# yukara-ikemiya/friendly-stable-audio-tools

Measured on AMD Instinct MI355X. Metric: audio-seconds/sec @44.1kHz stereo, 100-step DPM++, SA-Open-1.0 shape, higher is better.
Workload: dtype fp16; 1 GPU; Stable-Audio-Open-1.0 DiT shape (24 layers, D=1536, S=1025, CFG 7 -> 2 sequences/prompt) + Oobleck decode, 1 prompt(s)/GPU x 47.55 s, 100 DPM-Solver++(3M) SDE steps; prompts_per_gpu=1, codec_dtype=fp16, sampler_steps=100, layernorm=fused, cross_attention=fused, sample_size=2097152, parallelism=dp1 (rank-strided prompts, one all-gather)

## Files before the change

friendly-stable-audio-tools_amd/csrc/gemm_ph8.hip:

```cpp
#include <algorithm>
#include <type_traits>

#include "sat_common.h"

namespace {

typedef __attribute__((address_space(3))) void* lds_void_p;
typedef float f32x4_t __attribute__((ext_vector_type(4)));

template <int N>
__device__ __forceinline__ void wait_lgkmcnt() {
    asm volatile("s_waitcnt lgkmcnt(%0)" ::"n"(N) : "memory");
}

__device__ __forceinline__ float silu_fast(float x) { return x * __builtin_amdgcn_rcpf(1.0f + __expf(-x)); }

__device__ __forceinline__ unsigned lds_addr(const void* p) {
    return (unsigned)(size_t)(__attribute__((address_space(3))) const char*)(const char*)p;
}
__device__ __forceinline__ float lds_ld32(const void* p) {
    float v;
    asm volatile("ds_read_b32 %0, %1" : "=v"(v) : "v"(lds_addr(p)) : "memory");
    return v;
}
// ... 4 lines not shown
}
__device__ __forceinline__ f32x4_t lds_ld128(const void* p) {
    f32x4_t v;
    asm volatile("ds_read_b128 %0, %1" : "=v"(v) : "v"(lds_addr(p)) : "memory");
    return v;
}
__device__ __forceinline__ void lds_st64(void* p, float2 v) { asm volatile("ds_write_b64 %0, %1" ::"v"(lds_addr(p)), "v"(v) : "memory"); }
__device__ __forceinline__ void lds_st128(void* p, f32x4_t v) { asm volatile("ds_write_b128 %0, %1" ::"v"(lds_addr(p)), "v"(v) : "memory"); }
__device__ __forceinline__ void lds_tie() {}
template <typename T, typename... Ts>
__device__ __forceinline__ void lds_tie(T& v, Ts&... vs) {
    asm volatile("" : "+v"(v));
    lds_tie(vs...);
}
template <typename... Ts>
__device__ __forceinline__ void lds_wait(Ts&... vs) {
    asm volatile("s_waitcnt lgkmcnt(0)" ::: "memory");
    lds_tie(vs...);
}

template <int PERM>
__device__ __forceinline__ int chan_of(int ni, int nf, int i) {
    const int q = i >> 2, r = i & 3;
    if constexpr (PERM == 0) return ni * 32 + nf * 16 + i;
    else if constexpr (PERM == 1) return ni * 32 + q * 8 + nf * 4 + r;
    else return ni == 0 ? nf * 16 + i : 32 + q * 8 + nf * 4 + r;
}

struct Seg {
    int m0, n0;
    int kt0, nk;
    bool whole;
    bool tr;
};

struct Ph8F32Epi {
    __amdgpu_buffer_rsrc_t rsC, rsXb, rsPart;
    int ldc, N;
    bool accumulate, prod;
    const float* gate;
    int gate_rows, gate_ld, M;
};
__device__ __forceinline__ Ph8F32Epi ph8_f32_epi(const GemmArgs& g) {
    Ph8F32Epi e;
    e.rsC = __builtin_amdgcn_make_buffer_rsrc((void*)g.C, 0, (int)((unsigned)g.M * (unsigned)g.ldc * 4u), 0x00020000);
    e.rsXb = __builtin_amdgcn_make_buffer_rsrc((void*)g.xb, 0, g.xb ? (int)((unsigned)g.M * (unsigned)g.N * 2u) : 0, 0x00020000);
    e.rsPart = __builtin_amdgcn_make_buffer_rsrc((void*)g.ln_part_out, 0, g.ln_part_out ? (int)((unsigned)g.M * (unsigned)(g.N >> 6) * 8u) : 0, 0x00020000);
    e.ldc = g.ldc; e.N = g.N; e.accumulate = g.accumulate != 0; e.prod = g.xb != nullptr;
    e.gate = g.gate; e.gate_rows = g.gate_rows; e.gate_ld = g.gate_ld; e.M = g.M;
    return e;
}
typedef unsigned int ph8_u32x4 __attribute__((ext_vector_type(4)));
typedef unsigned int ph8_u32x2 __attribute__((ext_vector_type(2)));
__device__ __forceinline__ void ph8_load_resid(const Ph8F32Epi& e, f32x4_t (&old)[4], int m, int ncol0, int q4) {
    const int off = (m * e.ldc + ncol0 + 4 * q4) * 4;
#pragma unroll
    for (int nb = 0; nb < 4; ++nb)
        old[nb] = __builtin_bit_cast(f32x4_t, __builtin_amdgcn_raw_buffer_load_b128(e.rsC, off + nb * 64, 0, 0));
}
template <bool RT, bool PROD_C>
__device__ __forceinline__ void ph8_epi_f32_row(const Ph8F32Epi& e, f32x4_t (&v)[4], const f32x4_t (&old)[4], int m, int ncol0, int q4) {
    const int off = (m * e.ldc + ncol0 + 4 * q4) * 4;
    [[maybe_unused]] const float* grow = nullptr;
    bool prod = PROD_C;
    if constexpr (RT) {
        prod = e.prod;
// ... 6 lines not shown
#pragma unroll
    for (int nb = 0; nb < 4; ++nb) {
        f32x4_t x = v[nb];
        if constexpr (RT) {
            if (grow) x *= *reinterpret_cast<const f32x4_t*>(grow + nb * 16);
        }
        const f32x4_t o = old[nb];
        x += e.accumulate ? o : f32x4_t{0.f, 0.f, 0.f, 0.f};
        __builtin_amdgcn_raw_buffer_store_b128(__builtin_bit_cast(ph8_u32x4, x), e.rsC, off + nb * 64, 0, 0);
        if (prod) {
            opx4 xr;
#pragma unroll
            for (int k = 0; k < 4; ++k) {
                xr[k] = f32_to_op(x[k]);
                const float f = op_to_f32(xr[k]);
                sum += f;
                sq += f * f;
            }
            __builtin_amdgcn_raw_buffer_store_b64(__builtin_bit_cast(ph8_u32x2, xr), e.rsXb, (m * e.N + ncol0 + 4 * q4 + nb * 16) * 2, 0, 0);
        }
    }
    if (prod) {
        sum += __int_as_float(__builtin_amdgcn_ds_swizzle(__float_as_int(sum), 0x401F));
        sq += __int_as_float(__builtin_amdgcn_ds_swizzle(__float_as_int(sq), 0x401F));
        u32x2 a = __builtin_amdgcn_permlane32_swap(__float_as_uint(sum), __float_as_uint(sum), false, false);
        u32x2 b = __builtin_amdgcn_permlane32_swap(__float_as_uint(sq), __float_as_uint(sq), false, false);
        sum = __uint_as_float(a[0]) + __uint_as_float(a[1]);
        sq = __uint_as_float(b[0]) + __uint_as_float(b[1]);
        const int poff = q4 == 0 ? (m * (e.N >> 6) + (ncol0 >> 6)) * 8 : 0x7ffffff0;
        __builtin_amdgcn_raw_buffer_store_b64(ph8_u32x2{__float_as_uint(sum), __float_as_uint(sq)}, e.rsPart, poff, 0, 0);
    }
}

template <int EPI, int DBG = 0, int FP8 = 0, bool GATED = false>
__global__ __launch_bounds__(512) void gemm_ph8_kernel(GemmArgs g, Ph8Sched sc, unsigned long long* ts = nullptr) {
    sat_f16_saturate();
    constexpr int WN = 4, MFQ = 4;
    constexpr int NW = 2 * WN, NT = NW * 64;
    constexpr int QR = MFQ * 16;
    constexpr int WR = 2 * QR;
    constexpr int BM = 2 * WR, BN = WN * 64;
    constexpr int MB = 2 * MFQ;
    constexpr int AH = (BM / 2) * 128, WH = (BN / 2) * 128;
    static_assert(NT / 2 == BM, "two threads per row in the LayerNorm prologue");
    [[maybe_unused]] int ts_n = 0;
    constexpr int BUF_BYTES = 2 * (AH + WH), RING_BYTES = 2 * BUF_BYTES;
    auto koff = [](int kind) { return kind == 0 ? 0 : kind == 1 ? WH : kind == 2 ? WH + AH : 2 * WH + AH; };
    extern __shared__ __attribute__((aligned(16))) char smem[];

    const int tid_ = threadIdx.x;
    const int lane = tid_ & 63;
    const int wave = __builtin_amdgcn_readfirstlane(tid_ >> 6);
    const int wr = wave / WN, wc = wave % WN;
    const int l15_ = lane & 15, q4_ = lane >> 4;
    const int M = g.M, N = g.N, K = g.K;
    const int wgi = xcd_remap(blockIdx.x, sc.G);

    auto tile_of = [&](int id, int& tm, int& tn) { ph8_tile_of(sc, id, tm, tn); };
    int dp_s = 0;
    int sk_b = 0, sk_e = 0;
    if (sc.sk_tiles) ph8_wg_units(sc, wgi, sk_b, sk_e);
    int sk_u = sk_b;
    auto next_seg = [&](Seg& s) -> bool {
        int tm, tn;
        if (dp_s < sc.dp_rounds) {
            tile_of(dp_s * sc.G + wgi, tm, tn);
            ++dp_s;
            s.kt0 = 0; s.nk = 2 * sc.nkp; s.whole = true;
        } else {
            if (sk_u >= sk_e) return false;
            const int j = sk_u / sc.nkp;
            const int ub = sk_u - j * sc.nkp;
            const int ue = min(sc.nkp, ub + (sk_e - sk_u));
            tile_of(sc.rem0 + j, tm, tn);
            s.kt0 = 2 * ub; s.nk = 2 * (ue - ub); s.whole = (ub == 0 && ue == sc.nkp);
            sk_u += ue - ub;
        }
        s.m0 = tm * BM; s.n0 = tn * BN;
        s.tr = true;
        if constexpr (EPI == EPI_HEADS) s.tr = !(g.heads.kind[s.n0 / (g.heads.heads * 64)] & 1);
        return true;
    };

    const __amdgpu_buffer_rsrc_t rsA = __builtin_amdgcn_make_buffer_rsrc((void*)g.A, 0, (int)((unsigned)M * (unsigned)K * 2u), 0x00020000);
    __amdgpu_buffer_rsrc_t rsW = rsA;
    int voffA[2], voffW[2][2];
    auto setup_dma = [&](const Seg& s) {
        int lane_l = lane;
        asm volatile("" : "+v"(lane_l));
        rsW = __builtin_amdgcn_make_buffer_rsrc((void*)(g.W + (size_t)s.n0 * K), 0, BN * K * 2, 0x00020000);
        const int sub = lane_l >> 3, pos = lane_l & 7;
#pragma unroll
        for (int i = 0; i < 2; ++i) {
            const int r = i * (NW * 8) + wave * 8 + sub;
            const int c = pos ^ ((r >> 1) & 7);
            voffA[i] = (s.m0 + (r / QR) * WR + (r % QR)) * (K * 2) + c * 16;
            const int wcol = r >> 5, nf = (r >> 4) & 1, fi = r & 15;
#pragma unroll
            for (int ni = 0; ni < 2; ++ni) {
                int ch;
                if constexpr (EPI == EPI_F32) ch = chan_of<0>(ni, nf, fi);
                else if constexpr (EPI == EPI_SWIGLU) ch = chan_of<1>(ni, nf, fi);
                else ch = s.tr ? chan_of<2>(ni, nf, fi) : chan_of<0>(ni, nf, fi);
                voffW[ni][i] = (wcol * 64 + ch) * (K * 2) + c * 16;
            }
        }
    };
    const int hiA = QR * K * 2;
    auto issue = [&](int kind, int buf, int kt) {
        char* dst = smem + buf * BUF_BYTES + koff(kind) + wave * 1024;
        const int soff = __builtin_amdgcn_readfirstlane(kt * 128);
#pragma unroll
        for (int i = 0; i < 2; ++i) {
            if (kind & 1)
                __builtin_amdgcn_raw_ptr_buffer_load_lds(rsA, (lds_void_p)(dst + i * (NW * 1024)), 16, voffA[i] + (kind == 3 ? hiA : 0), soff, 0, 0);
            else
                __builtin_amdgcn_raw_ptr_buffer_load_lds(rsW, (lds_void_p)(dst + i * (NW * 1024)), 16, voffW[kind >> 1][i], soff, 0, 0);
        }
    };

    const int swz = l15_ >> 1;
    [[maybe_unused]] const int swz_ = swz;
    int offA[2], offW[2];
#pragma unroll
    for (int ks = 0; ks < 2; ++ks) {
        const int ch = ((ks * 4 + q4_) ^ swz) << 4;
        offA[ks] = (wr * QR + l15_) * 128 + ch;
        offW[ks] = (wc * 32 + l15_) * 128 + ch;
    }

    f32x4_t acc[MB][4];
    opx8 fa[MFQ][2], fwl[2][2], fwh[2][2];
    typedef int i32x8_t __attribute__((ext_vector_type(8)));
    [[maybe_unused]] i32x8_t fa8[MFQ], fw8l[2], fw8h[2];
    [[maybe_unused]] const int off8[2] = {(((2 * q4_) ^ swz_) << 4), (((2 * q4_ + 1) ^ swz_) << 4)};
    auto read8 = [&](const char* rowbase) -> i32x8_t {
        const u32x4 lo = *reinterpret_cast<const u32x4*>(rowbase + off8[0]);
        const u32x4 hi = *reinterpret_cast<const u32x4*>(rowbase + off8[1]);
        return i32x8_t{(int)lo[0], (int)lo[1], (int)lo[2], (int)lo[3], (int)hi[0], (int)hi[1], (int)hi[2], (int)hi[3]};
    };
    [[maybe_unused]] auto read_a8 = [&](int buf, int hi) {
        const char* base = smem + buf * BUF_BYTES + koff(hi ? 3 : 1) + (wr * QR + l15_) * 128;
#pragma unroll
        for (int f = 0; f < MFQ; ++f) fa8[f] = read8(base + f * 2048);
    };
    [[maybe_unused]] auto read_w8 = [&](int buf, int hi, i32x8_t (&fw)[2]) {
        const char* base = smem + buf * BUF_BYTES + koff(hi ? 2 : 0) + (wc * 32 + l15_) * 128;
#pragma unroll
        for (int f = 0; f < 2; ++f) fw[f] = read8(base + f * 2048);
    };
    auto read_a = [&](int buf, int hi) {
        const char* base = smem + buf * BUF_BYTES + koff(hi ? 3 : 1);
#pragma unroll
        for (int f = 0; f < MFQ; ++f)
#pragma unroll
            for (int ks = 0; ks < 2; ++ks) fa[f][ks] = *reinterpret_cast<const opx8*>(base + offA[ks] + f * 2048);
    };
    auto read_w = [&](int buf, int hi, opx8 (&fw)[2][2]) {
        const char* base = smem + buf * BUF_BYTES + koff(hi ? 2 : 0);
#pragma unroll
        for (int f = 0; f < 2; ++f)
#pragma unroll
            for (int ks = 0; ks < 2; ++ks) fw[f][ks] = *reinterpret_cast<const opx8*>(base + offW[ks] + f * 2048);
    };

    auto main_loop = [&](auto swap_c, const int kt0, const int nk, const bool q_valid0, const bool q_valid1) {
        constexpr bool SWAP = decltype(swap_c)::value;
        auto mfma_half = [&](int mi, int ni_first) {
            if (!(mi ? q_valid1 : q_valid0)) return;
            __builtin_amdgcn_s_setprio(1);
            if constexpr (FP8 != 0) {
#pragma unroll
                for (int h = 0; h < 2; ++h) {
                    const int ni = ni_first ^ h;
                    i32x8_t (&fw)[2] = ni ? fw8h : fw8l;
#pragma unroll
                    for (int f = 0; f < MFQ; ++f)
#pragma unroll
                        for (int n = 0; n < 2; ++n)
                            acc[mi * MFQ + f][ni * 2 + n] =
                                SWAP ? __builtin_amdgcn_mfma_scale_f32_16x16x128_f8f6f4(fw[n], fa8[f], acc[mi * MFQ + f][ni * 2 + n], 0, 0, 0, 0x7F7F7F7F, 0, 0x7F7F7F7F)
                                     : __builtin_amdgcn_mfma_scale_f32_16x16x128_f8f6f4(fa8[f], fw[n], acc[mi * MFQ + f][ni * 2 + n], 0, 0, 0, 0x7F7F7F7F, 0, 0x7F7F7F7F);
                }
                __builtin_amdgcn_s_setprio(0);
                return;
            }
#pragma unroll
            for (int h = 0; h < 2; ++h) {
                const int ni = ni_first ^ h;
                opx8 (&fw)[2][2] = ni ? fwh : fwl;
#pragma unroll
                for (int ks = 0; ks < 2; ++ks)
#pragma unroll
                    for (int f = 0; f < MFQ; ++f)
#pragma unroll
                        for (int n = 0; n < 2; ++n)
                            acc[mi * MFQ + f][ni * 2 + n] = SWAP ? mfma_16x16x32(fw[n][ks], fa[f][ks], acc[mi * MFQ + f][ni * 2 + n])
                                                                 : mfma_16x16x32(fa[f][ks], fw[n][ks], acc[mi * MFQ + f][ni * 2 + n]);
            }
            __builtin_amdgcn_s_setprio(0);
        };
        auto k_tile = [&](auto buf_c, auto mode_c, int t) {
            constexpr int BUF = decltype(buf_c)::value;
            constexpr int MODE = decltype(mode_c)::value;
            if constexpr (FP8 != 0) {
                read_w8(BUF, 0, fw8l);
                read_w8(BUF, 1, fw8h);
                read_a8(BUF, 0);
            } else {
                read_w(BUF, 0, fwl);
                read_w(BUF, 1, fwh);
                read_a(BUF, 0);
            }
            if constexpr (MODE <= 1) {
                issue(2, BUF ^ 1, t + 1);
                issue(3, BUF ^ 1, t + 1);
                wait_vmcnt<8>();
            } else {
                wait_vmcnt<0>();
            }
            __builtin_amdgcn_sched_barrier(0);
            wait_lgkmcnt<0>();
            __builtin_amdgcn_s_barrier();
            __builtin_amdgcn_sched_barrier(0);
            mfma_half(0, 0);
            __builtin_amdgcn_sched_barrier(0);
            __builtin_amdgcn_s_barrier();
            if constexpr (FP8 != 0) read_a8(BUF, 1);
            else read_a(BUF, 1);
            if constexpr (MODE == 0) {
                issue(0, BUF, t + 2);
                issue(1, BUF, t + 2);
                wait_vmcnt<6>();
// ... 113 lines not shown

    struct RopePre {
        f32x4_t cs, sn;
    };
    constexpr int ROPE16_OFF = RING_BYTES + 2 * LN_BYTES;
    if constexpr (EPI == EPI_HEADS) {
        if (tid_ < 32 && g.heads.rope_cos) {
            const int r16 = g.heads.S > 16 ? 16 : g.heads.S - 1;
            reinterpret_cast<float*>(smem + ROPE16_OFF)[tid_] = (tid_ < 16 ? g.heads.rope_cos : g.heads.rope_sin)[r16 * 16 + (tid_ & 15)];
        }
    }
    constexpr int PRO_DMA = 2 * (4 + PRO_T1);
    static_assert(PRO_DMA == 12, "prologue = 6 half-tiles");
    [[maybe_unused]] auto rope_load = [&](f32x4_t& cs, f32x4_t& sn, int row, int q4) {
        const unsigned voff = (unsigned)(row * 16 + 4 * q4) * 4u;
        asm volatile("global_load_dwordx4 %0, %1, %2" : "=v"(cs) : "v"(voff), "s"(g.heads.rope_cos) : "memory");
        asm volatile("global_load_dwordx4 %0, %1, %2" : "=v"(sn) : "v"(voff), "s"(g.heads.rope_sin) : "memory");
    };
    [[maybe_unused]] auto rope_prefetch = [&](const Seg& s, RopePre& rp) {
        int l15 = l15_, q4 = q4_;
        asm volatile("" : "+v"(l15), "+v"(q4));
        const int S = g.heads.S;
        const int m = s.m0 + wr * WR + l15;
        rope_load(rp.cs, rp.sn, (m < M ? m : M - 1) % S, q4);
    };
    [[maybe_unused]] auto rope_wait = [](auto n_c, RopePre& rp) {
        wait_vmcnt<decltype(n_c)::value>();
        asm volatile("" : "+v"(rp.cs), "+v"(rp.sn));
    };

    auto epilogue = [&](const Seg& s, int lb, [[maybe_unused]] RopePre& rp, [[maybe_unused]] const bool dma_behind) {
        int l15 = l15_, q4 = q4_;
        asm volatile("" : "+v"(l15), "+v"(q4));
        const int mrow0 = s.m0 + wr * WR + l15;
        const int ncol0 = s.n0 + wc * 64;
        [[maybe_unused]] const float2* ln = reinterpret_cast<const float2*>(smem + RING_BYTES + lb * LN_BYTES) + wr * WR;
        [[maybe_unused]] const float* lc1 = reinterpret_cast<const float*>(smem + RING_BYTES + lb * LN_BYTES + BM * 8) + wc * 64;
        [[maybe_unused]] const float* lc2 = lc1 + BN;
        if constexpr (EPI == EPI_F32) {
            const Ph8F32Epi fe = ph8_f32_epi(g);
            auto run = [&](auto rt_c, auto prod_c) {
                constexpr bool RT = decltype(rt_c)::value, PROD = decltype(prod_c)::value;
                f32x4_t old[2][2][4];
#pragma unroll
                for (int i = 0; i < 2; ++i) ph8_load_resid(fe, old[0][i], mrow0 + i * 16, ncol0, q4);
#pragma unroll
                for (int h = 0; h < MB / 2; ++h) {
                    if (h + 1 < MB / 2) {
#pragma unroll
                        for (int i = 0; i < 2; ++i) ph8_load_resid(fe, old[(h + 1) & 1][i], mrow0 + ((h + 1) * 2 + i) * 16, ncol0, q4);
                    }
                    __builtin_amdgcn_sched_barrier(0);
#pragma unroll
                    for (int i = 0; i < 2; ++i) ph8_epi_f32_row<RT, PROD>(fe, acc[h * 2 + i], old[h & 1][i], mrow0 + (h * 2 + i) * 16, ncol0, q4);
                    __builtin_amdgcn_sched_barrier(0);
                }
            };
            if constexpr (GATED) run(std::true_type{}, std::false_type{});
            else run(std::false_type{}, std::true_type{});
        } else if constexpr (EPI == EPI_SWIGLU) {
            const int ldh = N >> 1;
            f32x4_t c1v[2], c1g[2], c2v[2], c2g[2];
#pragma unroll
            for (int nf = 0; nf < 2; ++nf) {
                c1v[nf] = lds_ld128(lc1 + q4 * 8 + nf * 4);
                c1g[nf] = lds_ld128(lc1 + 32 + q4 * 8 + nf * 4);
                c2v[nf] = lds_ld128(lc2 + q4 * 8 + nf * 4);
                c2g[nf] = lds_ld128(lc2 + 32 + q4 * 8 + nf * 4);
            }
            float2 stv[MB];
#pragma unroll
            for (int mb = 0; mb < MB; ++mb) stv[mb] = lds_ld64(ln + mb * 16 + l15);
            lds_wait(c1v[0], c1v[1], c1g[0], c1g[1], c2v[0], c2v[1], c2g[0], c2g[1]);
#pragma unroll
            for (int mb = 0; mb < MB; ++mb) lds_tie(stv[mb]);
            const __amdgpu_buffer_rsrc_t rsH = __builtin_amdgcn_make_buffer_rsrc((void*)g.H, 0, (int)((unsigned)M * (unsigned)ldh * 2u), 0x00020000);
            const int hcol = (ncol0 >> 1) + q4 * 8;
#pragma unroll
            for (int mb = 0; mb < MB; ++mb) {
                const int m = mrow0 + mb * 16;
                const float2 st = stv[mb];
                unsigned pk[4];
                [[maybe_unused]] float hv8[8];
#pragma unroll
                for (int nf = 0; nf < 2; ++nf) {
                    float hv[4];
#pragma unroll
                    for (int e = 0; e < 4; ++e) {
                        const float v = fold(acc[mb][nf][e], st.x, st.y, c1v[nf][e], c2v[nf][e]);
                        const float gt = fold(acc[mb][2 + nf][e], st.x, st.y, c1g[nf][e], c2g[nf][e]);
                        hv[e] = v * silu_fast(gt);
                        if constexpr (FP8 != 0) hv8[4 * nf + e] = hv[e];
                    }
                    pk[2 * nf] = pack_op2(hv[0], hv[1]);
                    pk[2 * nf + 1] = pack_op2(hv[2], hv[3]);
                }
                if constexpr (FP8 != 0) {
                    if (g.H8) {
                        float am = 0.f;
#pragma unroll
                        for (int i = 0; i < 8; ++i) am = fmaxf(am, fabsf(hv8[i]));
                        am = m < M ? am : 0.f;
                        am = fmaxf(am, __int_as_float(__builtin_amdgcn_ds_swizzle(__float_as_int(am), 0x401F)));
                        am = fmaxf(am, __int_as_float(__builtin_amdgcn_ds_bpermute((lane ^ 32) << 2, __float_as_int(am))));
                        const float t = am * (1.0f / 448.0f);
                        const unsigned tb = __float_as_uint(t);
                        int e = (int)((tb >> 23) & 0xff) - 127 + ((tb & 0x7fffff) ? 1 : 0);
                        e = am > 0.f ? (e < -127 ? -127 : (e > 127 ? 127 : e)) : -127;
                        const float inv = __uint_as_float((unsigned)(127 - e) << 23);
                        unsigned q0 = __builtin_amdgcn_cvt_pk_fp8_f32(hv8[0] * inv, hv8[1] * inv, 0u, false);
                        q0 = __builtin_amdgcn_cvt_pk_fp8_f32(hv8[2] * inv, hv8[3] * inv, q0, true);
                        unsigned q1 = __builtin_amdgcn_cvt_pk_fp8_f32(hv8[4] * inv, hv8[5] * inv, 0u, false);
                        q1 = __builtin_amdgcn_cvt_pk_fp8_f32(hv8[6] * inv, hv8[7] * inv, q1, true);
                        if (m < M) {
                            *reinterpret_cast<u32x2*>(g.H8 + (size_t)m * ldh + (ncol0 >> 1) + q4 * 8) = u32x2{q0, q1};
                            if (q4 == 0) g.Hs[(size_t)m * (ldh >> 5) + (ncol0 >> 6)] = (unsigned char)(e + 127);
                        }
                        continue;
                    }
                }
                __builtin_amdgcn_raw_buffer_store_b128(ph8_u32x4{pk[0], pk[1], pk[2], pk[3]}, rsH, (m * ldh + hcol) * 2, 0, 0);
            }
        } else {
            const HeadsEpi& he = g.heads;
            const int hp = he.heads * 64;
            const int part = ncol0 / hp;
            const int head = (ncol0 - part * hp) >> 6;
            const int kind = he.kind[part];
            op_t* __restrict__ dst = he.out[part];
            const int S = he.S, Spad = he.Spad;
            if (s.tr) {
                f32x4_t c1[4], c2[4];
#pragma unroll
                for (int nf = 0; nf < 2; ++nf) {
                    c1[nf] = lds_ld128(lc1 + nf * 16 + 4 * q4);
                    c2[nf] = lds_ld128(lc2 + nf * 16 + 4 * q4);
                    c1[2 + nf] = lds_ld128(lc1 + 32 + q4 * 8 + nf * 4);
                    c2[2 + nf] = lds_ld128(lc2 + 32 + q4 * 8 + nf * 4);
                }
                float2 stv[2];
                stv[0] = lds_ld64(ln + l15);
                [[maybe_unused]] f32x4_t c16 = lds_ld128(smem + ROPE16_OFF + 16 * q4), s16 = lds_ld128(smem + ROPE16_OFF + 64 + 16 * q4);
                lds_wait(c1[0], c1[1], c1[2], c1[3], c2[0], c2[1], c2[2], c2[3], c16, s16, stv[0]);
                int b = 0, sq_ = 0;
                {
                    const int mc = mrow0 < M ? mrow0 : M - 1;
                    b = mc / S;
                    sq_ = mc - b * S;
                }
                if (kind & 2) {
                    if (dma_behind) rope_wait(std::integral_constant<int, PRO_DMA>{}, rp);
                    else rope_wait(std::integral_constant<int, 0>{}, rp);
                }
#pragma unroll
// ... 113 lines not shown
    prepare_finish(cur, lb, lnpre);
    while (true) {
        {
            f32x4_t b0[4] = {{0.f, 0.f, 0.f, 0.f}, {0.f, 0.f, 0.f, 0.f}, {0.f, 0.f, 0.f, 0.f}, {0.f, 0.f, 0.f, 0.f}};
            if constexpr (EPI == EPI_F32) {
                if (g.bias && cur.whole) {
                    int q4 = q4_;
                    asm volatile("" : "+v"(q4));
#pragma unroll
                    for (int j = 0; j < 4; ++j) b0[j] = *reinterpret_cast<const f32x4_t*>(g.bias + cur.n0 + wc * 64 + 4 * q4 + j * 16);
                }
            }
#pragma unroll
            for (int i = 0; i < MB; ++i)
#pragma unroll
                for (int j = 0; j < 4; ++j) acc[i][j] = b0[j];
        }
        if constexpr (EPI != EPI_HEADS) {
#pragma unroll
            for (int i = 0; i < MB; ++i)
#pragma unroll
                for (int j = 0; j < 4; ++j) asm volatile("" : "+v"(acc[i][j]));
        }
        if constexpr (EPI_STORES >= 0) {
            if (stores_behind) wait_vmcnt<6 + (EPI_STORES >= 0 ? EPI_STORES : 0)>();
            else wait_vmcnt<6>();
        } else {
            wait_vmcnt<0>();
        }
        wait_lgkmcnt<0>();
        __builtin_amdgcn_s_barrier();
        [[maybe_unused]] unsigned long long t0 = 0, t1 = 0, t2 = 0;
        if constexpr (DBG == 9) t0 = __builtin_amdgcn_s_memrealtime();
        const int mq = cur.m0 + wr * WR;
        const bool rows_valid = mq < M;
        if (cur.tr) main_loop(std::true_type{}, cur.kt0, cur.nk, rows_valid, mq + QR < M);
        else main_loop(std::false_type{}, cur.kt0, cur.nk, rows_valid, mq + QR < M);
        if constexpr (DBG == 9) t1 = __builtin_amdgcn_s_memrealtime();
        const bool more = next_seg(nxt);
        [[maybe_unused]] RopePre rp;
        if constexpr (EPI == EPI_HEADS) {
            if (rows_valid && cur.tr && (g.heads.kind[cur.n0 / (g.heads.heads * 64)] & 2)) rope_prefetch(cur, rp);
        }
        if (more) {
            prepare_issue(nxt, lnpre);
            if constexpr (!LN_DEFER) prepare_finish(nxt, lb ^ 1, lnpre);
        }
        bool fin = true;
        if (EPI == EPI_F32 && !cur.whole) {
            int lane_l = lane;
            asm volatile("" : "+v"(lane_l));
            float* mine = sc.sk_slab + (size_t)wgi * (BM * BN) + (size_t)(wave * MB * 4) * 256 + lane_l * 4;
#pragma unroll
            for (int mb = 0; mb < MB; ++mb)
#pragma unroll
                for (int nb = 0; nb < 4; ++nb) *reinterpret_cast<f32x4_t*>(mine + (mb * 4 + nb) * 256) = acc[mb][nb];
            fin = false;
        }
        if constexpr (DBG == 9) t2 = __builtin_amdgcn_s_memrealtime();
        if (fin && rows_valid) epilogue(cur, lb, rp, more);
        stores_behind = fin && rows_valid;
        if constexpr (DBG == 9) {
            if (tid_ == 0 && ts_n < 4) {
                unsigned long long* o = ts + ((size_t)blockIdx.x * 4 + ts_n) * 8;
                o[0] = t0; o[1] = t1; o[2] = t2; o[3] = __builtin_amdgcn_s_memrealtime();
                o[4] = cur.whole; o[5] = cur.nk; o[6] = fin; o[7] = 1;
            }
            ++ts_n;
        }
        if (!more) break;
// ... 9 lines not shown
    int first, parts;
    ph8_tile_parts(sc, j, first, parts);
    if (parts <= 1) return;
    const int tid = threadIdx.x, lane = tid & 63, wave = tid >> 6;
    const int wr = wave >> 2, wc = wave & 3, l15 = lane & 15, q4 = lane >> 4;
    int tm, tn;
    ph8_tile_of(sc, sc.rem0 + j, tm, tn);
    const int m = (tm << 8) + wr * 128 + mb * 16 + l15;
    const int ncol0 = (tn << 8) + wc * 64;
    if ((tm << 8) + wr * 128 >= g.M) return;
    f32x4_t v[4] = {{0.f, 0.f, 0.f, 0.f}, {0.f, 0.f, 0.f, 0.f}, {0.f, 0.f, 0.f, 0.f}, {0.f, 0.f, 0.f, 0.f}};
    for (int w = first; w < first + parts; ++w) {
        const float* src = sc.sk_slab + (size_t)w * 65536 + (size_t)(wave * 32 + mb * 4) * 256 + lane * 4;
#pragma unroll
        for (int nb = 0; nb < 4; ++nb) v[nb] += *reinterpret_cast<const f32x4_t*>(src + nb * 256);
    }
    f32x4_t bia[4];
#pragma unroll
    for (int nb = 0; nb < 4; ++nb)
        bia[nb] = g.bias ? *reinterpret_cast<const f32x4_t*>(g.bias + ncol0 + 4 * q4 + nb * 16) : f32x4_t{0.f, 0.f, 0.f, 0.f};
#pragma unroll
    for (int nb = 0; nb < 4; ++nb) v[nb] += bia[nb];
    f32x4_t old[4];
    const Ph8F32Epi fe = ph8_f32_epi(g);
    ph8_load_resid(fe, old, m, ncol0, q4);
    ph8_epi_f32_row<true, false>(fe, v, old, m, ncol0, q4);
}

int ph8_cus(int& out) {
    out = sat_device_cus();
    return out > 0 ? 0 : SAT_E_INVALID;
}

int ph8_schedule(const GemmArgs& a, bool epi_f32, int bm, int bn, int wgs_per_cu, Ph8Sched& s) {
    int cus = 0;
    SAT_TRY(ph8_cus(cus));
    const int split = sat_variant_split(a.variant);
    const bool have_slab = a.slab != nullptr && (split >= 0 || a.slab_bytes >= (size_t)cus * 65536 * sizeof(float));
    const int balance = sat_variant_has(a.variant, SAT_VARIANT_BALANCE_OFF) ? PH8_BALANCE_OFF : PH8_BALANCE_TWO_ROUNDS;
    const long used = ph8_schedule_ints(a.M, a.N, a.K, split, epi_f32, bm, bn, wgs_per_cu, cus, have_slab, balance, s);
    SAT_CHECK_ARG(used == 0, SAT_E_INVALID, "gemm(8-phase): the K-split needs %ld workgroups, has %d", used, s.G);
    if (s.split) {
        const size_t need = (size_t)s.G * 65536 * sizeof(float);
        SAT_CHECK_ARG(a.slab && a.slab_bytes >= need, SAT_E_WORKSPACE, "gemm(8-phase): the K-split of the remainder round needs %zu bytes of slab workspace, got %zu",
                      need, a.slab ? a.slab_bytes : (size_t)0);
        SAT_CHECK_ARG(((uintptr_t)a.slab & 15) == 0, SAT_E_INVALID, "gemm(8-phase): the slab workspace must be 16-byte aligned");
        s.sk_slab = a.slab;
    }
    return 0;
}

#ifdef SAT_GEMM_EXPERIMENTS
unsigned long long* g_ts_buf = nullptr;
#endif

template <int EPI, int DBG = 0, int FP8 = 0, bool GATED = false>
int launch_ph8(const GemmArgs& a0, hipStream_t stream) {
    GemmArgs a = a0;
    if constexpr (FP8 != 0) {
        SAT_CHECK_ARG(a0.fp8 == 2 && a0.K % 256 == 0 && a0.a_scale && a0.w_scale, SAT_E_UNSUPPORTED,
                      "gemm(8-phase, e4m3): K=%d must be a multiple of 256 and both scale vectors given", a0.K);
        SAT_CHECK_ARG(!a0.ln_part && (EPI == EPI_SWIGLU || !a0.H8), SAT_E_UNSUPPORTED, "gemm(8-phase, e4m3): no LayerNorm fold; MXFP8 output from SwiGLU only");
        a.K = a0.K / 2;
    } else {
        SAT_CHECK_ARG(!a.fp8 && !a.H8, SAT_E_UNSUPPORTED, "gemm(8-phase): built for bf16 operands");
    }
    constexpr int BM = 256, BN = 256, NT = 512;
    constexpr int LDS = 2 * 2 * (BM / 2 + BN / 2) * 128 + 2 * (BM + BN) * 8 + (EPI == EPI_HEADS ? 128 : 0);
    SAT_CHECK_ARG(a.N % BN == 0, SAT_E_UNSUPPORTED, "gemm(8-phase): N=%d not a multiple of %d", a.N, BN);
    SAT_CHECK_ARG(a.K % 128 == 0, SAT_E_UNSUPPORTED, "gemm(8-phase): K=%d must be a multiple of 128", a.K);
    SAT_CHECK_ARG((uint64_t)a.M * (uint64_t)a.K * 2u < (1ull << 31), SAT_E_UNSUPPORTED, "gemm(8-phase): A larger than 2 GiB");
    if constexpr (EPI == EPI_F32)
        SAT_CHECK_ARG(((uint64_t)a.M + 256) * (uint64_t)a.ldc * 4u < (1ull << 31) && a.ldc >= a.N, SAT_E_UNSUPPORTED, "gemm(8-phase): C larger than 2 GiB");
    if constexpr (EPI == EPI_SWIGLU)
        SAT_CHECK_ARG(((uint64_t)a.M + 256) * (uint64_t)(a.N / 2) * 2u < (1ull << 31), SAT_E_UNSUPPORTED, "gemm(8-phase): H larger than 2 GiB");
    constexpr bool LN_CONS = EPI == EPI_SWIGLU || EPI == EPI_HEADS;
    SAT_CHECK_ARG(LN_CONS || !a.ln_part, SAT_E_UNSUPPORTED, "gemm(8-phase): the LayerNorm fold is finished by the SwiGLU / heads epilogues");
    SAT_CHECK_ARG((!a.xb && !a.ln_part_out) || (EPI == EPI_F32 && a.xb && a.ln_part_out), SAT_E_UNSUPPORTED,
                  "gemm(8-phase): the bf16 image / row statistics come from the fp32-output epilogue");
    if constexpr (EPI == EPI_HEADS) {
        SAT_CHECK_ARG((a.heads.heads * 64) % BN == 0 && a.N == a.heads.parts * a.heads.heads * 64, SAT_E_UNSUPPORTED,
                      "gemm(8-phase): a %d-column tile must not straddle q / k / v (heads=%d)", BN, a.heads.heads);
        for (int p = 0; p < a.heads.parts; ++p)
            SAT_CHECK_ARG((a.heads.kind[p] & 3) != 3, SAT_E_UNSUPPORTED, "gemm(8-phase): no rotation on a transposed destination");
        SAT_CHECK_ARG(!a.heads.xa_k, SAT_E_UNSUPPORTED, "gemm(8-phase): the fused cross-attention epilogue lives in the 128 x 64 tile");
    }
    Ph8Sched sc;
    SAT_TRY(ph8_schedule(a, EPI == EPI_F32, BM, BN, 1, sc));
    SAT_CHECK_ARG(GATED == (a0.gate != nullptr), SAT_E_INVALID, "gemm(8-phase): gated / plain build mismatch");
    auto kern = gemm_ph8_kernel<EPI, DBG, FP8, GATED>;
    SAT_TRY(sat_ensure_dynamic_lds(reinterpret_cast<const void*>(kern), LDS));
    unsigned long long* ts = nullptr;
#ifdef SAT_GEMM_EXPERIMENTS
    if constexpr (DBG == 9) {
        if (!g_ts_buf) SAT_HIP(hipMalloc(&g_ts_buf, 256 * 4 * 8 * sizeof(unsigned long long)));
        SAT_HIP(hipMemsetAsync(g_ts_buf, 0, 256 * 4 * 8 * sizeof(unsigned long long), stream));
        ts = g_ts_buf;
    }
#endif
    hipLaunchKernelGGL(kern, dim3(sc.G), dim3(NT), LDS, stream, a, sc, ts);
    if (sc.split) hipLaunchKernelGGL(ph8_reduce_f32_kernel, dim3(sc.sk_tiles * 8), dim3(512), 0, stream, a, sc);
    SAT_LAUNCH_CHECK();
    return 0;
}

template <int EPI, int BUILD>
int launch_ph8_build(const GemmArgs& a, hipStream_t stream) {
    constexpr SatPh8Params p = sat_ph8_params(BUILD);
    return launch_ph8<EPI, p.dbg, p.fp8, p.gated>(a, stream);
}

template <int EPI>
int launch_ph8_epi(int build, const GemmArgs& a, hipStream_t stream) {
    switch (build) {
        case SAT_PH8_PLAIN: return launch_ph8_build<EPI, SAT_PH8_PLAIN>(a, stream);
        case SAT_PH8_GATED:
            if constexpr (EPI == EPI_F32) return launch_ph8_build<EPI, SAT_PH8_GATED>(a, stream);
            break;
#ifndef SAT_OPERAND_F16
        case SAT_PH8_E4M3:
            if constexpr (EPI != EPI_F32) return launch_ph8_build<EPI, SAT_PH8_E4M3>(a, stream);
            break;
#endif
// ... 37 lines not shown
```

friendly-stable-audio-tools_amd/csrc/gemm_tiles.h:

```cpp
#pragma once
#include <stdint.h>

#include "ph8_sched.h"

static inline int64_t round_up(int64_t x, int64_t m) { return (x + m - 1) / m * m; }
static inline int cdiv(int64_t a, int64_t b) { return (int)((a + b - 1) / b); }

enum {
    SAT_VARIANT_TILE = 0xff,
    SAT_VARIANT_CODE = 0xfff,
    SAT_VARIANT_FP8_PLAIN = 0x100,
    SAT_VARIANT_PACKED = 0x4000,
    SAT_VARIANT_SPLIT_FORCE = 0x10000,
    SAT_VARIANT_SPLIT_OFF = 0x20000,
    SAT_VARIANT_BALANCE_OFF = 0x200000,
    SAT_VARIANT_NO_KGROUP = 0x800000,
};
static inline int sat_variant_tile(int variant) { return variant & SAT_VARIANT_TILE; }
static inline int sat_variant_ph8_code(int variant) { return (variant & SAT_VARIANT_CODE) % 100; }
static inline int sat_variant_ablation(int variant) { return (variant & SAT_VARIANT_CODE) / 100; }
static inline bool sat_variant_has(int variant, int bit) { return (variant & bit) != 0; }
static inline int sat_variant_split(int variant) { return sat_variant_has(variant, SAT_VARIANT_SPLIT_FORCE) ? 1 : sat_variant_has(variant, SAT_VARIANT_SPLIT_OFF) ? 0 : -1; }

#define SAT_TILE_POLICY_SHIFT 24
static inline int sat_tile_policy_bits(int policy) { return (policy == 22 ? 1 : policy == 81 ? 2 : policy == 82 ? 3 : 0) << SAT_TILE_POLICY_SHIFT; }
static inline int sat_wide_tile_of(int variant) {
    const int p = (variant >> SAT_TILE_POLICY_SHIFT) & 7;
    return p == 1 ? 22 : p == 2 ? 81 : p == 3 ? 82 : 80;
}

enum SatGemmFamily {
    SAT_GEMM_NONE = 0,
    SAT_GEMM_REG,
    SAT_GEMM_DMA2,
    SAT_GEMM_PIPE,
    SAT_GEMM_PH8,
};
enum SatTileId {
    SAT_TILE_AUTO = 0,
    SAT_TILE_REF_128 = 1,
    SAT_TILE_DMA_128 = 5,
    SAT_TILE_128 = 15,
    SAT_TILE_128x64 = 16,
    SAT_TILE_256 = 22,
    SAT_TILE_256x192 = 30,
    SAT_TILE_128_DEEP = 44,
    SAT_TILE_128_KGROUP = 49,
    SAT_TILE_PH8 = 80,
    SAT_TILE_128x64_XATTN = 256,
// ... 184 lines not shown
```

friendly-stable-audio-tools_amd/csrc/ph8_sched.h:

```cpp
#pragma once

#ifdef __HIPCC__
#define SAT_HD __host__ __device__ __forceinline__
#else
#define SAT_HD inline
#endif

namespace {

SAT_HD int xcd_remap(int bid, int nwg) {
    const int NX = 8;
    int xcd = bid % NX, idx = bid / NX;
    int q = nwg / NX, r = nwg % NX;
    int base = (xcd < r) ? xcd * (q + 1) : r * (q + 1) + (xcd - r) * q;
    return base + idx;
}

struct Ph8Sched {
    int G;
    int tiles_n;
    int tiles_m_full;
    int light;
    int light_first;
    int dp_rounds;
    int nkp;
    int sk_tiles;
    int rem0;
    int split;
    int sk_q, sk_r;
    int cls_n[3], cls_p[3];
    float* sk_slab;
};

SAT_HD void ph8_wg_units(const Ph8Sched& sc, int i, int& b, int& e) {
    if (!sc.split) {
        const int lo = i < sc.sk_r ? i : sc.sk_r, hi = i + 1 < sc.sk_r ? i + 1 : sc.sk_r;
        b = (i * sc.sk_q + lo) * sc.nkp;
        e = ((i + 1) * sc.sk_q + hi) * sc.nkp;
        return;
    }
    int w0 = 0, j0 = 0;
    b = e = 0;
#pragma unroll
    for (int c = 0; c < 3; ++c) {
        const int n = sc.cls_n[c], p = sc.cls_p[c];
        if (i >= w0 && i < w0 + n * p) {
            const int j = j0 + (i - w0) / p, k = (i - w0) % p;
            b = j * sc.nkp + sc.nkp * k / p;
            e = j * sc.nkp + sc.nkp * (k + 1) / p;
        }
        w0 += n * p;
        j0 += n;
    }
}
SAT_HD void ph8_tile_parts(const Ph8Sched& sc, int j, int& first, int& parts) {
    int w0 = 0, j0 = 0;
    first = 0;
    parts = 1;
#pragma unroll
    for (int c = 0; c < 3; ++c) {
        const int n = sc.cls_n[c], p = sc.cls_p[c];
        if (j >= j0 && j < j0 + n) {
            first = w0 + (j - j0) * p;
            parts = p;
        }
        w0 += n * p;
        j0 += n;
    }
}

SAT_HD void ph8_tile_of(const Ph8Sched& sc, int id, int& tm, int& tn) {
    const int nl = sc.light ? sc.tiles_n : 0;
    const int lid = sc.light_first ? id : id - sc.tiles_m_full * sc.tiles_n;
    if (lid >= 0 && lid < nl) {
        tm = sc.tiles_m_full;
        tn = lid;
        return;
    }
    const int L = sc.light_first ? id - nl : id;
    const int tiles_m = sc.tiles_m_full, tiles_n = sc.tiles_n;
    if (tiles_m <= 12) {
        tn = L / tiles_m;
        tm = L - tn * tiles_m;
    } else {
        const int band_sz = 8 * tiles_n;
        const int band = L / band_sz;
        const int rem = L - band * band_sz;
        const int gm = tiles_m - band * 8 < 8 ? tiles_m - band * 8 : 8;
        tn = rem / gm;
        tm = band * 8 + (rem - tn * gm);
    }
}


inline bool ph8_auto_split(int M, int N, int K, bool epi_f32, int cus) {
    const long t_all = (long)((M + 255) / 256) * (N / 256);
    const long rem = t_all % cus;
    return epi_f32 && K >= 4096 && t_all > cus && rem > 0 && 2 * rem <= cus;
}

enum { PH8_BALANCE_TWO_ROUNDS = 0, PH8_BALANCE_OFF = 1 };

inline long ph8_schedule_ints(int M, int N, int K, int split, bool epi_f32, int bm, int bn, int wgs_per_cu, int cus, bool have_slab, int balance,
                              Ph8Sched& out) {
    auto lmin = [](long a, long b) { return a < b ? a : b; };
    auto lmax = [](long a, long b) { return a > b ? a : b; };
    if (split < 0) split = (bm == 256 && epi_f32 && have_slab && ph8_auto_split(M, N, K, epi_f32, cus)) ? 1 : 0;
    if (bm != 256 || !epi_f32) split = 0;
    Ph8Sched s{};
    const int tiles_m = (M + bm - 1) / bm, tail = M % bm;
    s.tiles_n = N / bn;
    s.light = (tail != 0 && tail <= bm / 4 && tiles_m > 1) ? 1 : 0;
    s.tiles_m_full = tiles_m - s.light;
    s.nkp = K / 128;
    const long t_full = (long)s.tiles_m_full * s.tiles_n, t_light = s.light ? s.tiles_n : 0;
    const long t_all = t_full + t_light;
    s.G = (int)lmin((long)cus * wgs_per_cu, split ? t_all * s.nkp : t_all);
    if (!split && !(balance & PH8_BALANCE_OFF) && t_all > s.G && t_all <= 2L * s.G) s.G = (int)((t_all + 1) / 2);
    s.dp_rounds = (int)((split ? t_all : t_full) / s.G);
    s.light_first = (split && s.dp_rounds >= 1 && t_light) ? 1 : 0;
    s.rem0 = (int)((long)s.dp_rounds * s.G);
    s.sk_tiles = (int)(t_all - s.rem0);
    s.split = (split && s.sk_tiles) ? 1 : 0;
    if (s.sk_tiles && !s.split) {
        s.sk_q = s.sk_tiles / s.G;
        s.sk_r = s.sk_tiles % s.G;
    } else if (s.sk_tiles) {
        const int n_light = s.light_first ? 0 : (int)lmin(t_light, s.sk_tiles);
        const int n_full = s.sk_tiles - n_light;
        const long cost2 = 2L * n_full + n_light;
        const int cap = s.nkp < 8 ? s.nkp : 8;
        const int pf = (int)lmax(1, lmin(cap, (long)s.G * 2 / cost2));
        const int pl = (int)lmax(1, lmin(cap, (long)s.G * 1 / cost2));
        long used = (long)n_full * pf + (long)n_light * pl;
        int extra = 0;
        if (pf < cap && used < s.G) extra = (int)lmin(n_full, s.G - used);
        used += extra;
        if (used > s.G) {
            out = s;
            return used;
        }
        s.cls_n[0] = extra; s.cls_p[0] = pf + 1;
        s.cls_n[1] = n_full - extra; s.cls_p[1] = pf;
        s.cls_n[2] = n_light; s.cls_p[2] = pl;
    }
    out = s;
    return 0;
}

}
```

Measured before the change: 75.75 audio-seconds/sec.

## Add half-row tile schedule for 16-bit SwiGLU GEMM to balance wave quantization

Adds a scheduling mode for the 256x256 SwiGLU GEMM. When the tile count lands between one and one-and-a-half rounds of CUs, some full tiles are split into two 128-row half tiles, and a 16-row tail is folded into the last half tile. Each workgroup then runs at most one full tile plus one half tile, which shortens the tail of a partly filled second round. The cost is a new templated kernel path with out-of-range buffer offsets that mask loads and stores. The mode is gated by a variant flag so it can be turned off.

```diff
diff --git a/friendly-stable-audio-tools_amd/csrc/gemm_ph8.hip b/friendly-stable-audio-tools_amd/csrc/gemm_ph8.hip
--- a/friendly-stable-audio-tools_amd/csrc/gemm_ph8.hip
+++ b/friendly-stable-audio-tools_amd/csrc/gemm_ph8.hip
@@ -60,6 +60,8 @@
     int kt0, nk;
     bool whole;
     bool tr;
+    bool half;
+    bool ext;
 };
 
 struct Ph8F32Epi {
@@ -132,7 +134,7 @@
     }
 }
 
-template <int EPI, int DBG = 0, int FP8 = 0, bool GATED = false>
+template <int EPI, int DBG = 0, int FP8 = 0, bool GATED = false, bool HRK = false>
 __global__ __launch_bounds__(512) void gemm_ph8_kernel(GemmArgs g, Ph8Sched sc, unsigned long long* ts = nullptr) {
     sat_f16_saturate();
     constexpr int WN = 4, MFQ = 4;
@@ -161,8 +163,37 @@
     int sk_b = 0, sk_e = 0;
     if (sc.sk_tiles) ph8_wg_units(sc, wgi, sk_b, sk_e);
     int sk_u = sk_b;
+    constexpr bool HR = HRK;
+    static_assert(!HRK || (EPI == EPI_SWIGLU && FP8 == 0 && DBG == 0), "half tiles: the 16-bit SwiGLU epilogue only");
+    [[maybe_unused]] int hr_step = 0;
     auto next_seg = [&](Seg& s) -> bool {
         int tm, tn;
+        s.half = s.ext = false;
+        if constexpr (HR) {
+            if (sc.hr) {
+                s.kt0 = 0; s.nk = 2 * sc.nkp; s.whole = true; s.tr = true;
+                if (hr_step == 0) {
+                    hr_step = 1;
+                    if (ph8_hr_has_full(sc, wgi)) {
+                        ph8_hr_full_of(sc, wgi, tm, tn);
+                        s.m0 = tm * BM; s.n0 = tn * BN;
+                        return true;
+                    }
+                }
+                if (hr_step == 1) {
+                    hr_step = 2;
+                    const int j = ph8_hr_half_index(sc, wgi);
+                    if (j >= 0) {
+                        int r0, ext;
+                        ph8_hr_half_of(sc, j, r0, tn, ext);
+                        s.m0 = r0; s.n0 = tn * BN;
+                        s.half = true; s.ext = ext != 0;
+                        return true;
+                    }
+                }
+                return false;
+            }
+        }
         if (dp_s < sc.dp_rounds) {
             tile_of(dp_s * sc.G + wgi, tm, tn);
             ++dp_s;
@@ -185,16 +216,27 @@
     const __amdgpu_buffer_rsrc_t rsA = __builtin_amdgcn_make_buffer_rsrc((void*)g.A, 0, (int)((unsigned)M * (unsigned)K * 2u), 0x00020000);
     __amdgpu_buffer_rsrc_t rsW = rsA;
     int voffA[2], voffW[2][2];
+    [[maybe_unused]] int voffAh[2];
+    const int hiA = QR * K * 2;
+    constexpr int VOFF_OOR = (int)0x80000000u;
     auto setup_dma = [&](const Seg& s) {
         int lane_l = lane;
         asm volatile("" : "+v"(lane_l));
         rsW = __builtin_amdgcn_make_buffer_rsrc((void*)(g.W + (size_t)s.n0 * K), 0, BN * K * 2, 0x00020000);
+        int wrs = WR;
+        if constexpr (HR) {
+            wrs = s.half ? QR : WR;
+        }
         const int sub = lane_l >> 3, pos = lane_l & 7;
 #pragma unroll
         for (int i = 0; i < 2; ++i) {
             const int r = i * (NW * 8) + wave * 8 + sub;
             const int c = pos ^ ((r >> 1) & 7);
-            voffA[i] = (s.m0 + (r / QR) * WR + (r % QR)) * (K * 2) + c * 16;
+            voffA[i] = (s.m0 + (r / QR) * wrs + (r % QR)) * (K * 2) + c * 16;
+            voffAh[i] = voffA[i] + QR * (K * 2);
+            if constexpr (HR) {
+                if (s.half && !(s.ext && r >= QR && r < QR + 16)) voffAh[i] = VOFF_OOR;
+            }
             const int wcol = r >> 5, nf = (r >> 4) & 1, fi = r & 15;
 #pragma unroll
             for (int ni = 0; ni < 2; ++ni) {
@@ -206,14 +248,13 @@
             }
         }
     };
-    const int hiA = QR * K * 2;
     auto issue = [&](int kind, int buf, int kt) {
         char* dst = smem + buf * BUF_BYTES + koff(kind) + wave * 1024;
         const int soff = __builtin_amdgcn_readfirstlane(kt * 128);
 #pragma unroll
         for (int i = 0; i < 2; ++i) {
             if (kind & 1)
-                __builtin_amdgcn_raw_ptr_buffer_load_lds(rsA, (lds_void_p)(dst + i * (NW * 1024)), 16, voffA[i] + (kind == 3 ? hiA : 0), soff, 0, 0);
+                __builtin_amdgcn_raw_ptr_buffer_load_lds(rsA, (lds_void_p)(dst + i * (NW * 1024)), 16, kind != 3 ? voffA[i] : HR ? voffAh[i] : voffA[i] + hiA, soff, 0, 0);
             else
                 __builtin_amdgcn_raw_ptr_buffer_load_lds(rsW, (lds_void_p)(dst + i * (NW * 1024)), 16, voffW[kind >> 1][i], soff, 0, 0);
         }
@@ -264,10 +305,9 @@
             for (int ks = 0; ks < 2; ++ks) fw[f][ks] = *reinterpret_cast<const opx8*>(base + offW[ks] + f * 2048);
     };
 
-    auto main_loop = [&](auto swap_c, const int kt0, const int nk, const bool q_valid0, const bool q_valid1) {
+    auto main_loop = [&](auto swap_c, const int kt0, const int nk, const bool q_valid0, const int q1_blocks) {
         constexpr bool SWAP = decltype(swap_c)::value;
-        auto mfma_half = [&](int mi, int ni_first) {
-            if (!(mi ? q_valid1 : q_valid0)) return;
+        auto mfma_blocks = [&](int mi, int ni_first, int nblk) {
             __builtin_amdgcn_s_setprio(1);
             if constexpr (FP8 != 0) {
 #pragma unroll
@@ -292,13 +332,21 @@
 #pragma unroll
                 for (int ks = 0; ks < 2; ++ks)
 #pragma unroll
-                    for (int f = 0; f < MFQ; ++f)
+                    for (int f = 0; f < nblk; ++f)
 #pragma unroll
                         for (int n = 0; n < 2; ++n)
                             acc[mi * MFQ + f][ni * 2 + n] = SWAP ? mfma_16x16x32(fw[n][ks], fa[f][ks], acc[mi * MFQ + f][ni * 2 + n])
                                                                  : mfma_16x16x32(fa[f][ks], fw[n][ks], acc[mi * MFQ + f][ni * 2 + n]);
             }
             __builtin_amdgcn_s_setprio(0);
+        };
+        auto mfma_half = [&](int mi, int ni_first) {
+            if (mi == 0) {
+                if (q_valid0) mfma_blocks(0, ni_first, MFQ);
+            } else {
+                if (q1_blocks == MFQ) mfma_blocks(1, ni_first, MFQ);
+                if (HR && q1_blocks == 1) mfma_blocks(1, ni_first, 1);
+            }
         };
         auto k_tile = [&](auto buf_c, auto mode_c, int t) {
             constexpr int BUF = decltype(buf_c)::value;
@@ -478,9 +526,10 @@
     auto epilogue = [&](const Seg& s, int lb, [[maybe_unused]] RopePre& rp, [[maybe_unused]] const bool dma_behind) {
         int l15 = l15_, q4 = q4_;
         asm volatile("" : "+v"(l15), "+v"(q4));
-        const int mrow0 = s.m0 + wr * WR + l15;
+        const int wrow = wr * ((HR && s.half) ? QR : WR);
+        const int mrow0 = s.m0 + wrow + l15;
         const int ncol0 = s.n0 + wc * 64;
-        [[maybe_unused]] const float2* ln = reinterpret_cast<const float2*>(smem + RING_BYTES + lb * LN_BYTES) + wr * WR;
+        [[maybe_unused]] const float2* ln = reinterpret_cast<const float2*>(smem + RING_BYTES + lb * LN_BYTES) + wrow;
         [[maybe_unused]] const float* lc1 = reinterpret_cast<const float*>(smem + RING_BYTES + lb * LN_BYTES + BM * 8) + wc * 64;
         [[maybe_unused]] const float* lc2 = lc1 + BN;
         if constexpr (EPI == EPI_F32) {
@@ -522,6 +571,13 @@
             for (int mb = 0; mb < MB; ++mb) lds_tie(stv[mb]);
             const __amdgpu_buffer_rsrc_t rsH = __builtin_amdgcn_make_buffer_rsrc((void*)g.H, 0, (int)((unsigned)M * (unsigned)ldh * 2u), 0x00020000);
             const int hcol = (ncol0 >> 1) + q4 * 8;
+            [[maybe_unused]] int off_q0 = 0, off_b4 = 0, off_q1 = 0;
+            if constexpr (HR) {
+                off_q0 = (mrow0 * ldh + hcol) * 2;
+                const int off_oor = 0x7ffffff0 - (MB - 1) * 16 * ldh * 2;
+                off_q1 = s.half ? off_oor : off_q0;
+                off_b4 = (s.half && !(s.ext && wr == 1)) ? off_oor : off_q0;
+            }
 #pragma unroll
             for (int mb = 0; mb < MB; ++mb) {
                 const int m = mrow0 + mb * 16;
@@ -565,7 +621,8 @@
                         continue;
                     }
                 }
-                __builtin_amdgcn_raw_buffer_store_b128(ph8_u32x4{pk[0], pk[1], pk[2], pk[3]}, rsH, (m * ldh + hcol) * 2, 0, 0);
+                __builtin_amdgcn_raw_buffer_store_b128(ph8_u32x4{pk[0], pk[1], pk[2], pk[3]}, rsH,
+                                                       HR ? (mb < MFQ ? off_q0 : mb == MFQ ? off_b4 : off_q1) + mb * 16 * ldh * 2 : (m * ldh + hcol) * 2, 0, 0);
             }
         } else {
             const HeadsEpi& he = g.heads;
@@ -745,10 +802,14 @@
         __builtin_amdgcn_s_barrier();
         [[maybe_unused]] unsigned long long t0 = 0, t1 = 0, t2 = 0;
         if constexpr (DBG == 9) t0 = __builtin_amdgcn_s_memrealtime();
-        const int mq = cur.m0 + wr * WR;
+        const int mq = cur.m0 + wr * ((HR && cur.half) ? QR : WR);
         const bool rows_valid = mq < M;
-        if (cur.tr) main_loop(std::true_type{}, cur.kt0, cur.nk, rows_valid, mq + QR < M);
-        else main_loop(std::false_type{}, cur.kt0, cur.nk, rows_valid, mq + QR < M);
+        int q1_blocks = mq + QR < M ? MFQ : 0;
+        if constexpr (HR) {
+            if (cur.half) q1_blocks = (cur.ext && wr == 1) ? 1 : 0;
+        }
+        if (cur.tr) main_loop(std::true_type{}, cur.kt0, cur.nk, rows_valid, q1_blocks);
+        else main_loop(std::false_type{}, cur.kt0, cur.nk, rows_valid, q1_blocks);
         if constexpr (DBG == 9) t1 = __builtin_amdgcn_s_memrealtime();
         const bool more = next_seg(nxt);
         [[maybe_unused]] RopePre rp;
@@ -824,9 +885,11 @@
     return out > 0 ? 0 : SAT_E_INVALID;
 }
 
-int ph8_schedule(const GemmArgs& a, bool epi_f32, int bm, int bn, int wgs_per_cu, Ph8Sched& s) {
+int ph8_schedule(const GemmArgs& a, bool epi_f32, bool swiglu16, int bm, int bn, int wgs_per_cu, Ph8Sched& s) {
     int cus = 0;
     SAT_TRY(ph8_cus(cus));
+    const bool hr_off = sat_variant_has(a.variant, SAT_VARIANT_HALF_ROWS_OFF) || sat_variant_has(a.variant, SAT_VARIANT_BALANCE_OFF);
+    if (bm == 256 && bn == 256 && wgs_per_cu == 1 && ph8_half_rows_ints(a.M, a.N, a.K, swiglu16, cus, hr_off, s)) return 0;
     const int split = sat_variant_split(a.variant);
     const bool have_slab = a.slab != nullptr && (split >= 0 || a.slab_bytes >= (size_t)cus * 65536 * sizeof(float));
     const int balance = sat_variant_has(a.variant, SAT_VARIANT_BALANCE_OFF) ? PH8_BALANCE_OFF : PH8_BALANCE_TWO_ROUNDS;
@@ -878,9 +941,12 @@
         SAT_CHECK_ARG(!a.heads.xa_k, SAT_E_UNSUPPORTED, "gemm(8-phase): the fused cross-attention epilogue lives in the 128 x 64 tile");
     }
     Ph8Sched sc;
-    SAT_TRY(ph8_schedule(a, EPI == EPI_F32, BM, BN, 1, sc));
+    SAT_TRY(ph8_schedule(a, EPI == EPI_F32, EPI == EPI_SWIGLU && FP8 == 0 && DBG == 0, BM, BN, 1, sc));
     SAT_CHECK_ARG(GATED == (a0.gate != nullptr), SAT_E_INVALID, "gemm(8-phase): gated / plain build mismatch");
     auto kern = gemm_ph8_kernel<EPI, DBG, FP8, GATED>;
+    if constexpr (EPI == EPI_SWIGLU && FP8 == 0 && DBG == 0) {
+        if (sc.hr) kern = gemm_ph8_kernel<EPI, DBG, FP8, GATED, true>;
+    }
     SAT_TRY(sat_ensure_dynamic_lds(reinterpret_cast<const void*>(kern), LDS));
     unsigned long long* ts = nullptr;
 #ifdef SAT_GEMM_EXPERIMENTS
diff --git a/friendly-stable-audio-tools_amd/csrc/gemm_tiles.h b/friendly-stable-audio-tools_amd/csrc/gemm_tiles.h
--- a/friendly-stable-audio-tools_amd/csrc/gemm_tiles.h
+++ b/friendly-stable-audio-tools_amd/csrc/gemm_tiles.h
@@ -15,6 +15,7 @@
     SAT_VARIANT_SPLIT_OFF = 0x20000,
     SAT_VARIANT_BALANCE_OFF = 0x200000,
     SAT_VARIANT_NO_KGROUP = 0x800000,
+    SAT_VARIANT_HALF_ROWS_OFF = 0x8000000,
 };
 static inline int sat_variant_tile(int variant) { return variant & SAT_VARIANT_TILE; }
 static inline int sat_variant_ph8_code(int variant) { return (variant & SAT_VARIANT_CODE) % 100; }
diff --git a/friendly-stable-audio-tools_amd/csrc/ph8_sched.h b/friendly-stable-audio-tools_amd/csrc/ph8_sched.h
--- a/friendly-stable-audio-tools_amd/csrc/ph8_sched.h
+++ b/friendly-stable-audio-tools_amd/csrc/ph8_sched.h
@@ -30,6 +30,10 @@
     int sk_q, sk_r;
     int cls_n[3], cls_p[3];
     float* sk_slab;
+    int hr;
+    int hr_full, hr_half;
+    int hr_q, hr_r;
+    int hr_ext;
 };
 
 SAT_HD void ph8_wg_units(const Ph8Sched& sc, int i, int& b, int& e) {
@@ -91,6 +95,38 @@
         tm = band * 8 + (rem - tn * gm);
     }
 }
+
+SAT_HD void ph8_hr_full_of(const Ph8Sched& sc, int L, int& tm, int& tn) {
+    const int fa = sc.tiles_m_full - sc.hr_q - 1, fb = fa + 1;
+    const int na = sc.hr_r * fa;
+    if (L < na) {
+        tn = L / fa;
+        tm = L - tn * fa;
+    } else {
+        const int c = (L - na) / fb;
+        tn = sc.hr_r + c;
+        tm = L - na - c * fb;
+    }
+}
+SAT_HD void ph8_hr_half_of(const Ph8Sched& sc, int j, int& r0, int& tn, int& ext) {
+    const int ha = 2 * (sc.hr_q + 1), hb = 2 * sc.hr_q;
+    const int na = sc.hr_r * ha;
+    int k, s;
+    if (j < na) {
+        tn = j / ha;
+        k = j - tn * ha;
+        s = sc.hr_q + 1;
+    } else {
+        const int c = (j - na) / hb;
+        tn = sc.hr_r + c;
+        k = j - na - c * hb;
+        s = sc.hr_q;
+    }
+    r0 = (sc.tiles_m_full - s) * 256 + k * 128;
+    ext = (sc.hr_ext && k == 2 * s - 1) ? 1 : 0;
+}
+SAT_HD bool ph8_hr_has_full(const Ph8Sched& sc, int wgi) { return wgi < sc.hr_full; }
+SAT_HD int ph8_hr_half_index(const Ph8Sched& sc, int wgi) { return wgi - (sc.G - sc.hr_half); }
 
 
 inline bool ph8_auto_split(int M, int N, int K, bool epi_f32, int cus) {
@@ -148,4 +184,28 @@
     return 0;
 }
 
-}
+inline bool ph8_half_rows_ints(int M, int N, int K, bool swiglu16, int cus, bool off, Ph8Sched& out) {
+    if (off || !swiglu16 || cus < 1 || M < 256 || N < 256 || N % 256 || K < 128 || K % 128) return false;
+    const int tail = M % 256;
+    if (tail > 16) return false;
+    const int tmf = M / 256, tiles_n = N / 256;
+    const long t = (long)tmf * tiles_n, G = cus;
+    if (!(t > G && 2 * t <= 3 * G)) return false;
+    const long S = (tail && t - G < tiles_n) ? tiles_n : t - G;
+    if (2 * S > G) return false;
+    Ph8Sched s{};
+    s.G = (int)G;
+    s.tiles_n = tiles_n;
+    s.tiles_m_full = tmf;
+    s.nkp = K / 128;
+    s.hr = 1;
+    s.hr_full = (int)(t - S);
+    s.hr_half = (int)(2 * S);
+    s.hr_q = (int)(S / tiles_n);
+    s.hr_r = (int)(S % tiles_n);
+    s.hr_ext = tail ? 1 : 0;
+    out = s;
+    return true;
+}
+
+}
```

New measurement: 76.79 audio-seconds/sec, median of 6. 1.4% higher.
